# hrz2000/CustomNeRF

Measured on AMD Instinct MI355X. Metric: training rays/s, higher is better.
Workload: dtype f16

## Files before the change

### customnerf_amd/csrc/gridencoder.hip

```cpp
#include "grid_common.h"

template <typename T, int D, int C>
__global__ void __launch_bounds__(GE_BLOCK) k_grid_fwd(const float *__restrict__ inputs, const T *__restrict__ grid, const GridLevels lv,
                                                       T *__restrict__ outputs, uint32_t B, uint32_t L, uint32_t n_levels, uint32_t nb,
                                                       T *__restrict__ dy_dx, uint32_t gridtype, int align_corners, uint32_t interp, int swizzle,
                                                       uint32_t ostride) {
    uint32_t level, pb;
    if (!ge_work_item(nb, n_levels, swizzle, lv, level, pb)) return;
    const uint32_t b = pb * GE_BLOCK + threadIdx.x;
    if (b >= B) return;

    using Vec = FeatVec<T, C>;
    const Vec *__restrict__ table = reinterpret_cast<const Vec *>(grid) + lv.offset[level];
    Vec *out = reinterpret_cast<Vec *>(outputs) + ((size_t)level * ostride + b);

    float in[D];
    bool oob = false;
    ge_load_coords<D>(inputs, b, in);
#pragma unroll
    for (int d = 0; d < D; d++) oob = oob || (in[d] < 0 || in[d] > 1);
    if (oob) {
        Vec z;
#pragma unroll
        for (int c = 0; c < C; c++) z.v[c] = ge_from_float<T>(0.0f);
        *out = z;
        if (dy_dx) {
            T *dd = dy_dx + (size_t)b * D * L * C + (size_t)level * D * C;
#pragma unroll
            for (int i = 0; i < D * C; i++) dd[i] = ge_from_float<T>(0.0f);
        }
        return;
    }

    const uint32_t hashmap_size = lv.size[level];
    const float scale = lv.scale[level];
    const uint32_t resolution = lv.resolution[level];

    float pos[D], pos_deriv[D];
    uint32_t pos_grid[D];
#pragma unroll
    for (int d = 0; d < D; d++) {
        pos[d] = cn_fma(in[d], scale, align_corners ? 0.0f : 0.5f);
        const float fl = floorf(pos[d]);
        pos_grid[d] = (uint32_t)fl;
        pos[d] -= (float)pos_grid[d];
        if (interp == 1) {
            pos_deriv[d] = ge_smoothstep_derivative(pos[d]);
            pos[d] = ge_smoothstep(pos[d]);
        } else {
            pos_deriv[d] = 1.0f;
        }
    }

    struct alignas(sizeof(T) * C) VecPair { Vec a, b; };
    struct alignas(sizeof(T) * C * 4) VecQuad { Vec e[4]; };
    Vec corner[1 << D];
    float wgt[1 << D];
    bool quad = false;
    if constexpr (sizeof(Vec) == 4) {
        quad = gridtype == 0 && ((lv.offset[level] | hashmap_size) & 3u) == 0 && ge_is_hashed<D>(align_corners, hashmap_size, resolution);
    }
    ge_dispatch_mode(ge_level_mode<D>(gridtype, align_corners, hashmap_size, resolution), [&](auto mode_c) {
#pragma unroll
    for (int q = 0; q < (1 << (D - 1)); q++) {
        uint32_t pgl[D];
#pragma unroll
        for (int d = 1; d < D; d++) pgl[d] = (((2 * q) & (1 << d)) == 0) ? pos_grid[d] : pos_grid[d] + 1;
        float w0 = 1 - pos[0], w1 = pos[0];
#pragma unroll
        for (int d = 1; d < D; d++) {
            const float f = (((2 * q) & (1 << d)) == 0) ? (1 - pos[d]) : pos[d];
            w0 *= f; w1 *= f;
        }
        wgt[2 * q] = w0; wgt[2 * q + 1] = w1;
        pgl[0] = pos_grid[0];
        const uint32_t i0 = ge_index_m<D, decltype(mode_c)::value>(gridtype, align_corners, hashmap_size, resolution, pgl);
        pgl[0] = pos_grid[0] + 1;
        const uint32_t i1 = ge_index_m<D, decltype(mode_c)::value>(gridtype, align_corners, hashmap_size, resolution, pgl);
        if (quad) {
            if constexpr (sizeof(Vec) == 4) {
                const VecQuad v = *reinterpret_cast<const VecQuad *>(table + (i0 & ~3u));
                const uint32_t k0 = i0 & 3u, k1 = i1 & 3u;
                const Vec a01 = (k0 & 1) ? v.e[1] : v.e[0], a23 = (k0 & 1) ? v.e[3] : v.e[2];
                corner[2 * q] = (k0 & 2) ? a23 : a01;
                const Vec b01 = (k1 & 1) ? v.e[1] : v.e[0], b23 = (k1 & 1) ? v.e[3] : v.e[2];
                Vec e1 = (k1 & 2) ? b23 : b01;
                if ((i0 ^ i1) > 3u) e1 = table[i1];
                corner[2 * q + 1] = e1;
            }
        } else {
            const uint32_t lo = min(i0, i1), hi_ = max(i0, i1);
            const uint32_t b = (lo + 1 < hashmap_size) ? lo : lo - 1;
            const VecPair v = *reinterpret_cast<const VecPair *>(table + b);
            const Vec e_lo = (b == lo) ? v.a : v.b;
            Vec e_hi = v.b;
            if (hi_ - lo != 1) e_hi = table[hi_];
            corner[2 * q] = (i0 == lo) ? e_lo : e_hi;
            corner[2 * q + 1] = (i0 == lo) ? e_hi : e_lo;
        }
    }
    });
    Vec res;
    if constexpr (sizeof(T) == 2 && C == 2) {
        __half2 r2 = __floats2half2_rn(0.0f, 0.0f);
#pragma unroll
        for (int idx = 0; idx < (1 << D); idx++) ge_accum2(r2, wgt[idx], *reinterpret_cast<const __half2 *>(&corner[idx]));
        res = *reinterpret_cast<const Vec *>(&r2);
    } else {
#pragma unroll
        for (int c = 0; c < C; c++) res.v[c] = ge_from_float<T>(0.0f);
#pragma unroll
        for (int idx = 0; idx < (1 << D); idx++) {
#pragma unroll
            for (int c = 0; c < C; c++) ge_accum(res.v[c], wgt[idx], corner[idx].v[c]);
        }
    }
    *out = res;

    if (dy_dx) {
        T *dd = dy_dx + (size_t)b * D * L * C + (size_t)level * D * C;
#pragma unroll
        for (int gd = 0; gd < D; gd++) {
            T rg[C];
#pragma unroll
            for (int c = 0; c < C; c++) rg[c] = ge_from_float<T>(0.0f);
#pragma unroll
            for (int idx = 0; idx < (1 << (D - 1)); idx++) {
                float w = scale;
                uint32_t pgl[D];
#pragma unroll
                for (int nd = 0; nd < D - 1; nd++) {
                    const int d = (nd >= gd) ? (nd + 1) : nd;
                    if ((idx & (1 << nd)) == 0) { w *= 1 - pos[d]; pgl[d] = pos_grid[d]; }
                    else { w *= pos[d]; pgl[d] = pos_grid[d] + 1; }
                }
                pgl[gd] = pos_grid[gd];
                const Vec left = table[ge_index<D>(gridtype, align_corners, hashmap_size, resolution, pgl)];
                pgl[gd] = pos_grid[gd] + 1;
                const Vec right = table[ge_index<D>(gridtype, align_corners, hashmap_size, resolution, pgl)];
#pragma unroll
                for (int c = 0; c < C; c++) {
                    if constexpr (sizeof(T) == 2) {
                        const float diff = __half2float(__float2half_rn(ge_opaque(__half2float(right.v[c]) - __half2float(left.v[c]))));
                        const float prod = ge_opaque(w * diff * pos_deriv[gd]);
                        rg[c] = __float2half_rn(ge_opaque(__half2float(rg[c]) + __half2float(__float2half_rn(prod))));
                    } else {
                        const float diff = right.v[c] - left.v[c];
                        rg[c] = cn_fma(w * diff, pos_deriv[gd], rg[c]);
                    }
                }
            }
#pragma unroll
            for (int c = 0; c < C; c++) dd[gd * C + c] = rg[c];
        }
    }
}

#include "grid_fwd_eval.h"

__global__ void __launch_bounds__(GE_BLOCK) k_grid_fwd_fast(const float *__restrict__ inputs, const __half *__restrict__ grid, const GridLevels lv,
                                                            __half *__restrict__ outputs, uint32_t B, uint32_t n_levels, uint32_t nb, uint32_t gridtype,
                                                            int swizzle, uint32_t ostride) {
    uint32_t level, pb;
    if (!ge_work_item(nb, n_levels, swizzle, lv, level, pb)) return;
    const uint32_t b = pb * GE_BLOCK + threadIdx.x;
    if (b >= B) return;
    uint32_t *out = reinterpret_cast<uint32_t *>(outputs) + ((size_t)level * ostride + b);
    float in[3];
    ge_load_coords<3>(inputs, b, in);
    if (in[0] < 0 || in[0] > 1 || in[1] < 0 || in[1] > 1 || in[2] < 0 || in[2] > 1) { *out = 0u; return; }

    const unsigned char *__restrict__ table = reinterpret_cast<const unsigned char *>(grid) + (size_t)lv.offset[level] * 4;
    *out = gf_eval_level(in, table, lv.size[level], lv.resolution[level], lv.scale[level], gridtype);
}

template <int SPT>
__global__ void __launch_bounds__(GE_BLOCK) k_grid_fwd_fast_sm(const float *__restrict__ inputs, const __half *__restrict__ grid, const GridLevels lv,
                                                               __half *__restrict__ outputs, uint32_t B, uint32_t n_levels, uint32_t gridtype,
                                                               uint32_t ostride) {
    const uint32_t t0 = blockIdx.x * (GE_BLOCK * SPT) + threadIdx.x;
    if (t0 >= B) return;
    float in[SPT][3];
    bool ok[SPT];
#pragma unroll
    for (int s = 0; s < SPT; s++) {
        ge_load_coords<3>(inputs, min(t0 + s * GE_BLOCK, B - 1), in[s]);
        ok[s] = !(in[s][0] < 0 || in[s][0] > 1 || in[s][1] < 0 || in[s][1] > 1 || in[s][2] < 0 || in[s][2] > 1);
#pragma unroll
        for (int d = 0; d < 3; d++) in[s][d] = ok[s] ? in[s][d] : 0.5f;
    }
    uint32_t *out = reinterpret_cast<uint32_t *>(outputs);
    for (uint32_t i = 0; i < n_levels; i++) {
        const uint32_t level = lv.order[i];
        const unsigned char *__restrict__ table = reinterpret_cast<const unsigned char *>(grid) + (size_t)lv.offset[level] * 4;
        const uint32_t size = lv.size[level], res = lv.resolution[level];
        const float scale = lv.scale[level];
#pragma unroll
        for (int s = 0; s < SPT; s++) {
            const uint32_t b = t0 + s * GE_BLOCK;
            const uint32_t r = gf_eval_level(in[s], table, size, res, scale, gridtype);
            if (b < B) out[(size_t)level * ostride + b] = ok[s] ? r : 0u;
        }
    }
}

template <typename T, int D, int C>
__global__ void __launch_bounds__(GE_BLOCK) k_grid_bwd(const T *__restrict__ grad, const float *__restrict__ inputs, const GridLevels lv,
                                                       float *__restrict__ grad_grid, uint32_t B, uint32_t n_levels, uint32_t nb,
                                                       uint32_t gridtype, int align_corners, uint32_t interp, int swizzle, float *__restrict__ found_inf) {
    uint32_t level, pb;
    if (!ge_work_item(nb, n_levels, swizzle, lv, level, pb)) return;
    const uint32_t b = pb * GE_BLOCK + threadIdx.x;
    if (b >= B) return;

    float in[D];
#pragma unroll
    for (int d = 0; d < D; d++) {
        in[d] = inputs[(size_t)b * D + d];
        if (!ge_in_range(in[d])) return;
    }
    using Vec = FeatVec<T, C>;
    const Vec g = reinterpret_cast<const Vec *>(grad)[(size_t)level * B + b];
    float *__restrict__ gtable = grad_grid + (size_t)lv.offset[level] * C;
    const uint32_t hashmap_size = lv.size[level];
    const float scale = lv.scale[level];
    const uint32_t resolution = lv.resolution[level];

    float pos[D];
    uint32_t pos_grid[D];
    ge_cell<D>(in, scale, align_corners, pos_grid, pos, interp);
    float gf[C];
#pragma unroll
    for (int c = 0; c < C; c++) {
        gf[c] = ge_to_float(g.v[c]);
        if (!(fabsf(gf[c]) <= 3.4e38f) && found_inf) *found_inf = 1.0f;
    }
#pragma unroll
    for (int idx = 0; idx < (1 << D); idx++) {
        float w;
        uint32_t entry;
        ge_corner<D>(idx, pos_grid, pos, gridtype, align_corners, hashmap_size, resolution, entry, w);
        const uint32_t index = entry * C;
#pragma unroll
        for (int c = 0; c < C; c++) unsafeAtomicAdd(&gtable[index + c], w * gf[c]);
    }
}

template <typename T, int D, int C>
__global__ void __launch_bounds__(GE_BLOCK) k_input_bwd(const T *__restrict__ grad, const T *__restrict__ dy_dx, float *__restrict__ grad_inputs,
                                                        uint32_t B, uint32_t L) {
    const uint32_t t = threadIdx.x + blockIdx.x * blockDim.x;
    if (t >= B * D) return;
    const uint32_t b = t / D, d = t - b * D;
    const T *dd = dy_dx + (size_t)b * L * D * C;
    float result = 0;
    for (uint32_t l = 0; l < L; l++) {
#pragma unroll
        for (int c = 0; c < C; c++)
            result = cn_fma(ge_to_float(grad[(size_t)l * B * C + (size_t)b * C + c]), ge_to_float(dd[l * D * C + d * C + c]), result);
    }
    grad_inputs[t] = result;
}

template <int D, int C>
__global__ void __launch_bounds__(GE_BLOCK) k_grad_tv(const float *__restrict__ inputs, const float *__restrict__ grid, float *__restrict__ grad,
                                                      const GridLevels lv, float weight, uint32_t B, uint32_t n_levels, uint32_t nb,
                                                      uint32_t gridtype, int align_corners) {
    uint32_t level, pb;
    if (!ge_work_item(nb, n_levels, 0, lv, level, pb)) return;
    const uint32_t b = pb * GE_BLOCK + threadIdx.x;
    if (b >= B) return;
    float in[D];
#pragma unroll
    for (int d = 0; d < D; d++) {
        in[d] = inputs[(size_t)b * D + d];
        if (!ge_in_range(in[d])) return;
    }
    const float *__restrict__ table = grid + (size_t)lv.offset[level] * C;
    float *__restrict__ gtable = grad + (size_t)lv.offset[level] * C;
    const uint32_t hashmap_size = lv.size[level], resolution = lv.resolution[level];
    const float scale = lv.scale[level];
    uint32_t pos_grid[D];
    float frac[D];
    ge_cell<D>(in, scale, align_corners, pos_grid, frac);
    float results[C], idelta[C];
#pragma unroll
    for (int c = 0; c < C; c++) { results[c] = 0; idelta[c] = 0; }
    const uint32_t index = ge_index<D>(gridtype, align_corners, hashmap_size, resolution, pos_grid) * C;
    const float w = weight / (2 * D);
#pragma unroll
    for (int d = 0; d < D; d++) {
        const uint32_t cur_d = pos_grid[d];
        if (cur_d < resolution) {
            pos_grid[d] = cur_d + 1;
            const uint32_t ir = ge_index<D>(gridtype, align_corners, hashmap_size, resolution, pos_grid) * C;
#pragma unroll
            for (int c = 0; c < C; c++) {
                const float gv = table[index + c] - table[ir + c];
                results[c] += gv;
                idelta[c] = cn_fma(gv, gv, idelta[c]);
            }
        }
        if (cur_d > 0) {
            pos_grid[d] = cur_d - 1;
            const uint32_t il = ge_index<D>(gridtype, align_corners, hashmap_size, resolution, pos_grid) * C;
#pragma unroll
            for (int c = 0; c < C; c++) {
                const float gv = table[index + c] - table[il + c];
                results[c] += gv;
                idelta[c] = cn_fma(gv, gv, idelta[c]);
            }
        }
        pos_grid[d] = cur_d;
    }
#pragma unroll
    for (int c = 0; c < C; c++) unsafeAtomicAdd(&gtable[index + c], w * results[c] * (1.0f / sqrtf(idelta[c] + 1e-9f)));
}

__global__ void __launch_bounds__(256) k_cast_f32_f16(const float *__restrict__ src, __half *__restrict__ dst, uint64_t n) {
    const uint64_t n8 = n / 8;
    const uint64_t stride = (uint64_t)gridDim.x * blockDim.x;
    for (uint64_t i = (uint64_t)blockIdx.x * blockDim.x + threadIdx.x; i < n8; i += stride) {
        const float4 a = reinterpret_cast<const float4 *>(src)[i * 2], b = reinterpret_cast<const float4 *>(src)[i * 2 + 1];
        union { __half2 h[4]; uint4 u; } o;
        o.h[0] = __floats2half2_rn(a.x, a.y);
        o.h[1] = __floats2half2_rn(a.z, a.w);
        o.h[2] = __floats2half2_rn(b.x, b.y);
        o.h[3] = __floats2half2_rn(b.z, b.w);
        reinterpret_cast<uint4 *>(dst)[i] = o.u;
    }
    for (uint64_t i = n8 * 8 + (uint64_t)blockIdx.x * blockDim.x + threadIdx.x; i < n; i += stride) dst[i] = __float2half_rn(src[i]);
}

static int ge_swizzle_default() {
    static const int v = cn_tune_env("CNERF_GRID_SWIZZLE", 2);
    return v;
}
static double ge_dense_weight() {
    static const double w = cn_tune_env_f("CNERF_GRID_DENSE_W", 0.7);
    return w;
}

static bool ge_fast_eligible(const GridLevels &lv, uint32_t nl, uint32_t gridtype) {
    static const int on = cn_tune_env("CNERF_GRID_FAST", 1);
    if (!on) return false;
    for (uint32_t l = 0; l < nl; l++) {
        const uint64_t step = (uint64_t)lv.resolution[l] + 1, cells = step * step * step;
        const uint32_t size = lv.size[l];
        const bool pow2 = (size & (size - 1)) == 0;
        if (size >= (1u << 24)) return false;
        if (cells <= size) continue;
        if (!pow2 || size < 8) return false;
        if (gridtype == 0 && ((lv.offset[l] | size) & 3u)) return false;
    }
    return true;
}

#define GE_TRAV_LEVEL 0u
#define GE_TRAV_SAMPLE 1u
#ifndef GE_FAST_SPT
#define GE_FAST_SPT 16
#endif

template <typename T, int D>
static int ge_fwd_C(const float *inputs, const T *emb, const GridLevels &lv, T *out, uint32_t B, uint32_t C, uint32_t L, uint32_t nl, T *dy_dx,
                    uint32_t gridtype, int ac, uint32_t interp, hipStream_t st, uint32_t ostride, uint32_t traversal = GE_TRAV_LEVEL) {
    uint32_t nb = cn_div_up(B, GE_BLOCK);
    const dim3 block(GE_BLOCK);
    int sw = ge_swizzle_default();
    if (sw == 2 && cn_tune_env("CNERF_GRID_SWIZZLE", -1) < 0) {
        uint64_t biggest = 0;
        for (uint32_t l = 0; l < nl; l++) biggest = biggest > lv.size[l] ? biggest : lv.size[l];
        if (biggest * C * sizeof(T) > (4ull << 20)) sw = 0;
    }
    GridLevels lvb = lv;
    if constexpr (std::is_same<T, __half>::value && D == 3) {
        if (C == 2 && !dy_dx && interp == 0 && !ac && ge_fast_eligible(lvb, nl, gridtype)) {
            static const int force = cn_tune_env("CNERF_GRID_TRAV", -1);
            if (force >= 0) traversal = (uint32_t)force;
            if (traversal == GE_TRAV_SAMPLE) {
                static const int spt = cn_tune_env("CNERF_GRID_SPT", GE_FAST_SPT);
#define GE_SM(SPT_) case SPT_: hipLaunchKernelGGL(k_grid_fwd_fast_sm<SPT_>, dim3(cn_div_up(B, GE_BLOCK * SPT_)), block, 0, st, inputs, emb, lvb, out, B, nl, gridtype, ostride); break;
                switch (spt) { GE_SM(4) GE_SM(8) GE_SM(32) default: GE_SM(16) }
#undef GE_SM
                return cn_launch_status();
            }
        }
    }
    dim3 grid(nb * nl);
    if (sw == 2) grid = dim3(CN_NXCD * ge_balance(lvb, nl, nb, D, gridtype, ac != 0, ge_dense_weight()));
    const GridLevels &lv_ = lvb;
    if constexpr (std::is_same<T, __half>::value && D == 3) {
        if (C == 2 && !dy_dx && interp == 0 && !ac && ge_fast_eligible(lv_, nl, gridtype)) {
            hipLaunchKernelGGL(k_grid_fwd_fast, grid, block, 0, st, inputs, emb, lv_, out, B, nl, nb, gridtype, sw, ostride);
            return cn_launch_status();
        }
    }
    switch (C) {
        case 1: hipLaunchKernelGGL((k_grid_fwd<T, D, 1>), grid, block, 0, st, inputs, emb, lv_, out, B, L, nl, nb, dy_dx, gridtype, ac, interp, sw, ostride); break;
        case 2: hipLaunchKernelGGL((k_grid_fwd<T, D, 2>), grid, block, 0, st, inputs, emb, lv_, out, B, L, nl, nb, dy_dx, gridtype, ac, interp, sw, ostride); break;
        case 4: hipLaunchKernelGGL((k_grid_fwd<T, D, 4>), grid, block, 0, st, inputs, emb, lv_, out, B, L, nl, nb, dy_dx, gridtype, ac, interp, sw, ostride); break;
        case 8: hipLaunchKernelGGL((k_grid_fwd<T, D, 8>), grid, block, 0, st, inputs, emb, lv_, out, B, L, nl, nb, dy_dx, gridtype, ac, interp, sw, ostride); break;
        default: return CNERF_EINVAL;
    }
    return cn_launch_status();
}

template <typename T>
static int ge_fwd_D(const float *inputs, const T *emb, const GridLevels &lv, T *out, uint32_t B, uint32_t D, uint32_t C, uint32_t L, uint32_t nl,
                    T *dy_dx, uint32_t gridtype, int ac, uint32_t interp, hipStream_t st, uint32_t ostride, uint32_t traversal = GE_TRAV_LEVEL) {
    switch (D) {
        case 2: return ge_fwd_C<T, 2>(inputs, emb, lv, out, B, C, L, nl, dy_dx, gridtype, ac, interp, st, ostride);
        case 3: return ge_fwd_C<T, 3>(inputs, emb, lv, out, B, C, L, nl, dy_dx, gridtype, ac, interp, st, ostride, traversal);
        case 4: return ge_fwd_C<T, 4>(inputs, emb, lv, out, B, C, L, nl, dy_dx, gridtype, ac, interp, st, ostride);
        case 5: return ge_fwd_C<T, 5>(inputs, emb, lv, out, B, C, L, nl, dy_dx, gridtype, ac, interp, st, ostride);
        default: return CNERF_EINVAL;
    }
}

template <typename T, int D>
static int ge_bwd_C(const T *grad, const float *inputs, const GridLevels &lv, float *gemb, uint32_t B, uint32_t C, uint32_t L, uint32_t nl,
                    const T *dy_dx, float *grad_inputs, uint32_t gridtype, int ac, uint32_t interp, hipStream_t st) {
    const uint32_t nb = cn_div_up(B, GE_BLOCK);
    const dim3 grid(nb * nl), block(GE_BLOCK);
    const int sw = ge_swizzle_default() ? 1 : 0;
    const dim3 gin(cn_div_up(B * D, GE_BLOCK));
    switch (C) {
        case 1:
            hipLaunchKernelGGL((k_grid_bwd<T, D, 1>), grid, block, 0, st, grad, inputs, lv, gemb, B, nl, nb, gridtype, ac, interp, sw, g_cn_found_inf);
            if (dy_dx) hipLaunchKernelGGL((k_input_bwd<T, D, 1>), gin, block, 0, st, grad, dy_dx, grad_inputs, B, L);
            break;
        case 2:
            hipLaunchKernelGGL((k_grid_bwd<T, D, 2>), grid, block, 0, st, grad, inputs, lv, gemb, B, nl, nb, gridtype, ac, interp, sw, g_cn_found_inf);
            if (dy_dx) hipLaunchKernelGGL((k_input_bwd<T, D, 2>), gin, block, 0, st, grad, dy_dx, grad_inputs, B, L);
            break;
        case 4:
            hipLaunchKernelGGL((k_grid_bwd<T, D, 4>), grid, block, 0, st, grad, inputs, lv, gemb, B, nl, nb, gridtype, ac, interp, sw, g_cn_found_inf);
            if (dy_dx) hipLaunchKernelGGL((k_input_bwd<T, D, 4>), gin, block, 0, st, grad, dy_dx, grad_inputs, B, L);
            break;
        case 8:
            hipLaunchKernelGGL((k_grid_bwd<T, D, 8>), grid, block, 0, st, grad, inputs, lv, gemb, B, nl, nb, gridtype, ac, interp, sw, g_cn_found_inf);
            if (dy_dx) hipLaunchKernelGGL((k_input_bwd<T, D, 8>), gin, block, 0, st, grad, dy_dx, grad_inputs, B, L);
            break;
        default: return CNERF_EINVAL;
    }
    return cn_launch_status();
}

template <typename T>
static int ge_bwd_D(const T *grad, const float *inputs, const GridLevels &lv, float *gemb, uint32_t B, uint32_t D, uint32_t C, uint32_t L,
                    uint32_t nl, const T *dy_dx, float *grad_inputs, uint32_t gridtype, int ac, uint32_t interp, hipStream_t st) {
    switch (D) {
        case 2: return ge_bwd_C<T, 2>(grad, inputs, lv, gemb, B, C, L, nl, dy_dx, grad_inputs, gridtype, ac, interp, st);
        case 3: return ge_bwd_C<T, 3>(grad, inputs, lv, gemb, B, C, L, nl, dy_dx, grad_inputs, gridtype, ac, interp, st);
        case 4: return ge_bwd_C<T, 4>(grad, inputs, lv, gemb, B, C, L, nl, dy_dx, grad_inputs, gridtype, ac, interp, st);
        case 5: return ge_bwd_C<T, 5>(grad, inputs, lv, gemb, B, C, L, nl, dy_dx, grad_inputs, gridtype, ac, interp, st);
        default: return CNERF_EINVAL;
    }
}

template <int D>
static int ge_tv_C(const float *inputs, const float *emb, float *grad, const GridLevels &lv, float weight, uint32_t B, uint32_t C, uint32_t L,
                   uint32_t gridtype, int ac, hipStream_t st) {
    const uint32_t nb = cn_div_up(B, GE_BLOCK);
    const dim3 grid(nb * L), block(GE_BLOCK);
    switch (C) {
        case 1: hipLaunchKernelGGL((k_grad_tv<D, 1>), grid, block, 0, st, inputs, emb, grad, lv, weight, B, L, nb, gridtype, ac); break;
        case 2: hipLaunchKernelGGL((k_grad_tv<D, 2>), grid, block, 0, st, inputs, emb, grad, lv, weight, B, L, nb, gridtype, ac); break;
        case 4: hipLaunchKernelGGL((k_grad_tv<D, 4>), grid, block, 0, st, inputs, emb, grad, lv, weight, B, L, nb, gridtype, ac); break;
        case 8: hipLaunchKernelGGL((k_grad_tv<D, 8>), grid, block, 0, st, inputs, emb, grad, lv, weight, B, L, nb, gridtype, ac); break;
        default: return CNERF_EINVAL;
    }
    return cn_launch_status();
}

bool bn_eligible(uint32_t B, uint32_t D, uint32_t C, uint32_t nl, const GridLevels &lv);
uint64_t bn_workspace_bytes(uint32_t B, uint32_t nl, const GridLevels &lv, int dtype);
int bn_backward(const void *grad, const float *inputs, const GridLevels &lv, float *gemb, uint32_t B, uint32_t nl, uint32_t gridtype, int ac,
                uint32_t interp, int dtype, void *workspace, hipStream_t st, bool prepared);
int bn_prepare(const float *inputs, const GridLevels &lv, uint32_t B, uint32_t nl, uint32_t gridtype, int ac, uint32_t interp, int dtype,
               void *workspace, hipStream_t st);
bool bn_needs_plan(uint32_t B, uint32_t nl, const GridLevels &lv, int dtype, uint32_t gridtype);
void bn_grid_adam_arm(const CnerfGridAdam *cfg);
int bn_grid_adam_consumed();
#define BN_MIN_UPDATES (1u << 20)

extern "C" {

int cnerf_grid_backward_adam(const CnerfGridAdam *cfg) {
    if (cfg) {
        if (!cfg->p || !cfg->g || !cfg->m || !cfg->v || !cfg->scaler_state) return CNERF_ENULL;
        if (cfg->n == 0 || (cfg->n & 3) || ((((uintptr_t)cfg->p) | ((uintptr_t)cfg->g) | ((uintptr_t)cfg->m) | ((uintptr_t)cfg->v)) & 15) ||
            (((uintptr_t)cfg->p_half) & 7))
            return CNERF_EINVAL;
        if (!(cfg->beta1 >= 0.0f && cfg->beta1 < 1.0f) || !(cfg->beta2 >= 0.0f && cfg->beta2 < 1.0f) || !(cfg->eps >= 0.0f)) return CNERF_EINVAL;
    }
    bn_grid_adam_arm(cfg);
    return CNERF_OK;
}

int cnerf_grid_backward_adam_consumed(int *yes) {
    if (!yes) return CNERF_ENULL;
    *yes = bn_grid_adam_consumed();
    return CNERF_OK;
}

int cnerf_grid_encode_forward_ordered(const float *inputs, const void *embeddings, const int32_t *offsets_host, void *outputs, uint32_t B, uint32_t D,
                                      uint32_t C, uint32_t L, uint32_t max_level, float S, uint32_t H, void *dy_dx, uint32_t gridtype, int align_corners,
                                      uint32_t interp, int dtype, uint32_t out_level_stride, uint32_t traversal, void *stream) {
    if (gridtype > 1 || interp > 1 || traversal > GE_TRAV_SAMPLE) return CNERF_EINVAL;
    GridLevels lv;
    const uint32_t nl = max_level < L ? max_level : L;
    int rc = ge_levels(offsets_host, L, nl, S, H, lv);
    if (rc) return rc;
    if (D < 2 || D > 5 || !(C == 1 || C == 2 || C == 4 || C == 8)) return CNERF_EINVAL;
    if (dtype != CNERF_F32 && dtype != CNERF_F16) return CNERF_EINVAL;
    if (out_level_stride == 0) out_level_stride = B;
    if (out_level_stride < B) return CNERF_EINVAL;
    if (B == 0 || nl == 0) return CNERF_OK;
    if (!inputs || !embeddings || !outputs) return CNERF_ENULL;
    if (dtype == CNERF_F32)
        return ge_fwd_D<float>(inputs, (const float *)embeddings, lv, (float *)outputs, B, D, C, L, nl, (float *)dy_dx, gridtype, align_corners, interp,
                               CN_STREAM(stream), out_level_stride);
    return ge_fwd_D<__half>(inputs, (const __half *)embeddings, lv, (__half *)outputs, B, D, C, L, nl, (__half *)dy_dx, gridtype, align_corners, interp,
                            CN_STREAM(stream), out_level_stride, traversal);
}

int cnerf_grid_encode_forward_strided(const float *inputs, const void *embeddings, const int32_t *offsets_host, void *outputs, uint32_t B, uint32_t D,
                                      uint32_t C, uint32_t L, uint32_t max_level, float S, uint32_t H, void *dy_dx, uint32_t gridtype, int align_corners,
                                      uint32_t interp, int dtype, uint32_t out_level_stride, void *stream) {
    return cnerf_grid_encode_forward_ordered(inputs, embeddings, offsets_host, outputs, B, D, C, L, max_level, S, H, dy_dx, gridtype, align_corners, interp,
                                             dtype, out_level_stride, GE_TRAV_LEVEL, stream);
}

int cnerf_grid_encode_forward(const float *inputs, const void *embeddings, const int32_t *offsets_host, void *outputs, uint32_t B, uint32_t D,
                              uint32_t C, uint32_t L, uint32_t max_level, float S, uint32_t H, void *dy_dx, uint32_t gridtype, int align_corners,
                              uint32_t interp, int dtype, void *stream) {
    return cnerf_grid_encode_forward_strided(inputs, embeddings, offsets_host, outputs, B, D, C, L, max_level, S, H, dy_dx, gridtype, align_corners, interp,
                                             dtype, B, stream);
}

int cnerf_grid_encode_backward_workspace_bytes(const int32_t *offsets_host, uint32_t B, uint32_t D, uint32_t C, uint32_t L, uint32_t max_level,
                                               float S, uint32_t H, int dtype, uint64_t *bytes) {
    if (!bytes) return CNERF_ENULL;
    *bytes = 0;
    GridLevels lv;
    const uint32_t nl = max_level < L ? max_level : L;
    int rc = ge_levels(offsets_host, L, nl, S, H, lv);
    if (rc) return rc;
    if (dtype != CNERF_F32 && dtype != CNERF_F16) return CNERF_EINVAL;
    if ((uint64_t)B * nl >= BN_MIN_UPDATES && bn_eligible(B, D, C, nl, lv)) *bytes = bn_workspace_bytes(B, nl, lv, dtype);
    return CNERF_OK;
}

int cnerf_grid_encode_backward(const void *grad, const float *inputs, const int32_t *offsets_host, float *grad_embeddings, uint32_t B, uint32_t D,
                               uint32_t C, uint32_t L, uint32_t max_level, float S, uint32_t H, const void *dy_dx, float *grad_inputs,
                               uint32_t gridtype, int align_corners, uint32_t interp, int dtype, void *workspace, uint64_t workspace_bytes,
                               void *stream) {
    if (gridtype > 1 || interp > 1) return CNERF_EINVAL;
    GridLevels lv;
    const uint32_t nl = max_level < L ? max_level : L;
    int rc = ge_levels(offsets_host, L, nl, S, H, lv);
    if (rc) return rc;
    if (D < 2 || D > 5 || !(C == 1 || C == 2 || C == 4 || C == 8)) return CNERF_EINVAL;
    if (dtype != CNERF_F32 && dtype != CNERF_F16) return CNERF_EINVAL;
    if (!grad_embeddings) return CNERF_ENULL;
    if (B == 0 || nl == 0) return CNERF_OK;
    if (!grad || !inputs) return CNERF_ENULL;
    if (dy_dx && !grad_inputs) return CNERF_ENULL;
    if (workspace && !dy_dx && (uint64_t)B * nl >= BN_MIN_UPDATES && bn_eligible(B, D, C, nl, lv) &&
        workspace_bytes >= bn_workspace_bytes(B, nl, lv, dtype) && !(((uintptr_t)workspace) & 255))
        return bn_backward(grad, inputs, lv, grad_embeddings, B, nl, gridtype, align_corners, interp, dtype, workspace, CN_STREAM(stream), false);
    if (dtype == CNERF_F32)
        return ge_bwd_D<float>((const float *)grad, inputs, lv, grad_embeddings, B, D, C, L, nl, (const float *)dy_dx, grad_inputs, gridtype, align_corners, interp, CN_STREAM(stream));
    if (dtype == CNERF_F16)
        return ge_bwd_D<__half>((const __half *)grad, inputs, lv, grad_embeddings, B, D, C, L, nl, (const __half *)dy_dx, grad_inputs, gridtype, align_corners, interp, CN_STREAM(stream));
    return CNERF_EINVAL;
}

int cnerf_grid_encode_backward_prepare(const float *inputs, const int32_t *offsets_host, uint32_t B, uint32_t D, uint32_t C, uint32_t L,
                                       uint32_t max_level, float S, uint32_t H, uint32_t gridtype, int align_corners, uint32_t interp, int dtype,
                                       void *workspace, uint64_t workspace_bytes, int *prepared, void *stream) {
    if (!prepared) return CNERF_ENULL;
    *prepared = 0;
    if (gridtype > 1 || interp > 1) return CNERF_EINVAL;
    GridLevels lv;
    const uint32_t nl = max_level < L ? max_level : L;
    int rc = ge_levels(offsets_host, L, nl, S, H, lv);
    if (rc) return rc;
    if (dtype != CNERF_F32 && dtype != CNERF_F16) return CNERF_EINVAL;
    if (B == 0 || nl == 0) return CNERF_OK;
    if (!inputs) return CNERF_ENULL;
    if (!(workspace && (uint64_t)B * nl >= BN_MIN_UPDATES && bn_eligible(B, D, C, nl, lv) && workspace_bytes >= bn_workspace_bytes(B, nl, lv, dtype) &&
          !(((uintptr_t)workspace) & 255)))
        return CNERF_OK;
    if (!bn_needs_plan(B, nl, lv, dtype, gridtype)) return CNERF_OK;
    rc = bn_prepare(inputs, lv, B, nl, gridtype, align_corners, interp, dtype, workspace, CN_STREAM(stream));
    if (rc == 0) *prepared = 1;
    return rc;
}

int cnerf_grid_encode_backward_needs_plan(const int32_t *offsets_host, uint32_t B, uint32_t D, uint32_t C, uint32_t L, uint32_t max_level, float S,
                                          uint32_t H, uint32_t gridtype, int dtype, int *needs_plan) {
    if (!needs_plan) return CNERF_ENULL;
    *needs_plan = 0;
    GridLevels lv;
    const uint32_t nl = max_level < L ? max_level : L;
    int rc = ge_levels(offsets_host, L, nl, S, H, lv);
    if (rc) return rc;
    if (dtype != CNERF_F32 && dtype != CNERF_F16) return CNERF_EINVAL;
    if (B && nl && (uint64_t)B * nl >= BN_MIN_UPDATES && bn_eligible(B, D, C, nl, lv) && bn_needs_plan(B, nl, lv, dtype, gridtype)) *needs_plan = 1;
    return CNERF_OK;
}

int cnerf_grid_encode_backward_prepared(const void *grad, const float *inputs, const int32_t *offsets_host, float *grad_embeddings, uint32_t B,
                                        uint32_t D, uint32_t C, uint32_t L, uint32_t max_level, float S, uint32_t H, uint32_t gridtype,
                                        int align_corners, uint32_t interp, int dtype, void *workspace, uint64_t workspace_bytes, void *stream) {
    if (gridtype > 1 || interp > 1) return CNERF_EINVAL;
    GridLevels lv;
    const uint32_t nl = max_level < L ? max_level : L;
    int rc = ge_levels(offsets_host, L, nl, S, H, lv);
    if (rc) return rc;
    if (dtype != CNERF_F32 && dtype != CNERF_F16) return CNERF_EINVAL;
    if (!grad_embeddings || !grad || !inputs || !workspace) return CNERF_ENULL;
    if (!((uint64_t)B * nl >= BN_MIN_UPDATES && bn_eligible(B, D, C, nl, lv) && workspace_bytes >= bn_workspace_bytes(B, nl, lv, dtype) &&
          !(((uintptr_t)workspace) & 255)))
        return CNERF_EINVAL;
    return bn_backward(grad, inputs, lv, grad_embeddings, B, nl, gridtype, align_corners, interp, dtype, workspace, CN_STREAM(stream), true);
}

int cnerf_grad_total_variation(const float *inputs, const float *embeddings, float *grad, const int32_t *offsets_host, float weight, uint32_t B,
                               uint32_t D, uint32_t C, uint32_t L, float S, uint32_t H, uint32_t gridtype, int align_corners, void *stream) {
    if (!inputs || !embeddings || !grad) return CNERF_ENULL;
    if (gridtype > 1) return CNERF_EINVAL;
    GridLevels lv;
    int rc = ge_levels(offsets_host, L, L, S, H, lv);
    if (rc) return rc;
    for (uint32_t l = 0; l < L; l++) lv.order[l] = (uint8_t)l;
    if (B == 0) return CNERF_OK;
    switch (D) {
        case 2: return ge_tv_C<2>(inputs, embeddings, grad, lv, weight, B, C, L, gridtype, align_corners, CN_STREAM(stream));
        case 3: return ge_tv_C<3>(inputs, embeddings, grad, lv, weight, B, C, L, gridtype, align_corners, CN_STREAM(stream));
        case 4: return ge_tv_C<4>(inputs, embeddings, grad, lv, weight, B, C, L, gridtype, align_corners, CN_STREAM(stream));
        case 5: return ge_tv_C<5>(inputs, embeddings, grad, lv, weight, B, C, L, gridtype, align_corners, CN_STREAM(stream));
        default: return CNERF_EINVAL;
    }
}

int cnerf_cast_f32_to_f16(const float *src, void *dst, uint64_t n, void *stream) {
    if (!src || !dst) return CNERF_ENULL;
    if (n == 0) return CNERF_OK;
    if ((((uintptr_t)src) & 15) || (((uintptr_t)dst) & 15)) return CNERF_EINVAL;
    const uint32_t blocks = (uint32_t)(cn_div_up64(cn_div_up64(n, 8), 256) < 2048 ? cn_div_up64(cn_div_up64(n, 8), 256) : 2048);
    hipLaunchKernelGGL(k_cast_f32_f16, dim3(blocks ? blocks : 1), dim3(256), 0, CN_STREAM(stream), src, (__half *)dst, n);
    return cn_launch_status();
}

}
```

### customnerf_amd/nerf/network_grid.py

```python
import torch
from torch import nn

from .renderer import NeRFRenderer
from .encoding import get_encoder, get_embedder
from .provider_utils import trunc_exp
from .. import tcnn
from ..field import field, field_attach, field_forward_raw, field_forward_rows, packed_weights
from ..gridencoder import GridEncoder


class RGB_network(nn.Module):

    def __init__(self, input_ch_views, opt=None):
        super().__init__()
        self.opt = opt
        cfg = {"otype": "FullyFusedMLP", "activation": "ReLU", "output_activation": "Sigmoid", "n_neurons": 64, "n_hidden_layers": 1}
        self.rgb_network = tcnn.Network(input_ch_views + 64, 3, cfg, seed=13)
        if getattr(opt, 'mask_no_dir', False):
            self.conf_network = tcnn.Network(64, 1, cfg, seed=14)
        else:
            ndim = 1 if getattr(opt, 'keyword2', None) is None else 2
            self.conf_network = tcnn.Network(input_ch_views + 64, ndim, cfg, seed=14)

    def forward(self, x):
        if getattr(self.opt, 'mask_no_dir', False):
            dir_dim = x.shape[-1] - 64
            _, fea = x.split([dir_dim, 64], dim=-1)
            rgb = self.rgb_network(x)
            rgb2 = self.conf_network(fea if getattr(self.opt, 'mask_no_dir_nodetach', False) else fea.detach())
        else:
            rgb = self.rgb_network(x)
            rgb2 = self.conf_network(x.detach())
        return torch.cat([rgb, rgb2], dim=-1)


class NeRFNetwork(NeRFRenderer):
    def __init__(self, opt, device=None, **unused):
        super().__init__(opt)
        grid_type = getattr(opt, 'grid_type', 'tiledgrid')
        self.pos_en, self.pos_en_dim = get_encoder(
            grid_type, input_dim=3,
            num_levels=getattr(opt, 'num_levels', 16), level_dim=getattr(opt, 'level_dim', 2),
            base_resolution=getattr(opt, 'base_resolution', 16),
            log2_hashmap_size=getattr(opt, 'log2_hashmap_size', 21),
            desired_resolution=getattr(opt, 'desired_resolution', 8192))
        n_geo = getattr(opt, 'n_hidden_geo', 2)
        self.network = tcnn.Network(self.pos_en_dim, 64, {"otype": "FullyFusedMLP", "activation": "ReLU", "output_activation": "None",
                                                          "n_neurons": 64, "n_hidden_layers": n_geo}, seed=10)
        self.density_network = tcnn.Network(64, 1, {"otype": "FullyFusedMLP", "activation": "ReLU", "output_activation": "None",
                                                    "n_neurons": 64, "n_hidden_layers": 1}, seed=11)
        self.dir_en, input_ch_views = get_embedder(4)
        sig = {"otype": "FullyFusedMLP", "activation": "ReLU", "output_activation": "Sigmoid", "n_neurons": 64, "n_hidden_layers": 1}
        if getattr(opt, 'train_conf', 0):
            if getattr(opt, 'detach_mask_from_field', False) or getattr(opt, 'mask_no_dir', False):
                self.rgb_network = RGB_network(input_ch_views, opt=opt)
            else:
                self.rgb_network = tcnn.Network(input_ch_views + 64, 3 + 1, sig, seed=12)
        else:
            self.rgb_network = tcnn.Network(input_ch_views + 64, 3, sig, seed=12)
        self.bg_net = None
        self.supports_dir_group = True

    def background(self, d):
        return torch.zeros(d.size(), dtype=d.dtype, device=d.device)

    def gaussian(self, x):
        d = (x ** 2).sum(-1)
        return 5 * torch.exp(-d / (2 * 0.2 ** 2))

    def _fused_cfg(self):
        cfg = getattr(self, '_fused_cfg_cache', None)
        if cfg is None:
            ok = (getattr(self.opt, 'fused_field', True) and isinstance(self.pos_en, GridEncoder) and self.pos_en.level_dim == 2
                  and self.pos_en.input_dim == 3 and self.pos_en.output_dim <= 64 and isinstance(self.rgb_network, tcnn.Network)
                  and self.network.n_hidden_layers in (1, 2) and self.density_network.n_hidden_layers == 1
                  and self.rgb_network.n_hidden_layers == 1 and self.rgb_network.n_output_dims in (3, 4))
            cfg = (self.pos_en.output_dim, self.network.n_hidden_layers, self.rgb_network.n_output_dims) if ok else False
            self._fused_cfg_cache = cfg
        return cfg

    def _half(self):
        return self.network.compute_dtype == torch.float16

    def _weight_image(self):
        if not self.__dict__.get('packed_field_weights') or not self._half():
            return None
        enc_dim, n_geo, n_rgb = self._fused_cfg()
        return packed_weights(self.__dict__.setdefault('_wimg_cache', {}), enc_dim, n_geo, n_rgb, self.network.params, self.density_network.params,
                              self.rgb_network.params)

    def _geo(self, x):
        x_en = self.pos_en(x, bound=self.opt.bound)
        fea = self.network(x_en)
        sigma = self.density_network(fea)
        sigma = trunc_exp(sigma.squeeze(-1) + self.gaussian(x))
        return fea, sigma

    def forward(self, x, d, l=None, ratio=1, shading='albedo', dir_group=1):
        cfg = self._fused_cfg()
        if cfg and x.is_cuda:
            enc_dim, n_geo, n_rgb = cfg
            x = x.reshape(-1, 3)
            enc = self.pos_en.encode(x, bound=self.opt.bound, half=self._half())
            sigma, rgbc = field(enc, x, d.reshape(-1, 3), dir_group, enc_dim, n_geo, n_rgb, self.network.params, self.density_network.params,
                                self.rgb_network.params, wimg=self._weight_image())
            return sigma, (rgbc if n_rgb == 4 else rgbc[:, :3]), None
        if dir_group != 1:
            d = d.reshape(-1, 3).repeat_interleave(dir_group, dim=0)[:x.reshape(-1, 3).shape[0]]
        fea, sigma = self._geo(x)
        view_en = self.dir_en(d)
        rgb_input = torch.cat([view_en.to(fea.dtype), fea], dim=-1)
        radiances = self.rgb_network(rgb_input)
        return sigma, radiances, None

    def density(self, x):
        cfg = self._fused_cfg()
        if cfg and x.is_cuda and not torch.is_grad_enabled():
            enc_dim, n_geo, n_rgb = cfg
            x = x.reshape(-1, 3).contiguous().float()
            enc = self.pos_en.encode(x, bound=self.opt.bound, half=self._half())
            sigma, _ = field_forward_raw(enc, x, None, 1, enc_dim, n_geo, n_rgb, self.network.params, self.density_network.params, None,
                                         with_rgb=False, wimg=self._weight_image())
            return {'sigma': sigma}
        return {'sigma': self._geo(x)[1]}

    @property
    def supports_split_eval(self):
        return bool(self._fused_cfg())

    def split_buffers(self, P, device):
        dt = torch.float16 if self._half() else torch.float32
        L = self.pos_en.num_levels
        return torch.empty(L, P, 2, dtype=dt, device=device), torch.empty(P, 3, dtype=torch.float32, device=device)

    @torch.no_grad()
    def split_encode(self, enc, unit, x, row0, unit_ready=False, importance=False):
        B = x.shape[0]
        u = unit[row0:row0 + B]
        if not unit_ready:
            torch.add(x, self.opt.bound, out=u)
            u.div_(2 * self.opt.bound)
        trav = 0
        if importance and getattr(self.opt, 'tune_gather_traversal', True):
            trav = self.__dict__.get('_fine_tuner')
            if trav is None:
                from ..gridencoder.grid import TraversalTuner
                trav = self.__dict__['_fine_tuner'] = TraversalTuner()
        self.pos_en.encode_into(u, enc, row0, half=self._half(), traversal=trav)

    @torch.no_grad()
    def split_density(self, enc, x):
        enc_dim, n_geo, n_rgb = self._fused_cfg()
        sigma, _ = field_forward_raw(enc, x, None, 1, enc_dim, n_geo, n_rgb, self.network.params, self.density_network.params, None, with_rgb=False,
                                     wimg=self._weight_image())
        return sigma

    def _overlap_plan(self):
        return getattr(self.opt, 'overlap_scatter_plan', True)

    def split_prepare(self, unit, grad_enabled):
        if not (grad_enabled and self.pos_en.embeddings.requires_grad and self._overlap_plan()):
            return None
        if not getattr(self.opt, 'early_scatter_plan', True):
            return None
        return self.pos_en.prepare_backward(unit, self._half())

    def split_forward(self, enc, unit, x, d, dir_group, plan=None):
        enc_dim, n_geo, n_rgb = self._fused_cfg()
        if torch.is_grad_enabled() and self.pos_en.embeddings.requires_grad:
            enc = self.pos_en.attach_backward(enc, unit, overlap=self._overlap_plan(), plan=plan)
        sigma, rgbc = field(enc, x, d.reshape(-1, 3), dir_group, enc_dim, n_geo, n_rgb, self.network.params, self.density_network.params,
                            self.rgb_network.params, grad_in_place=bool(getattr(self, 'grad_in_place', False)), wimg=self._weight_image())
        return sigma, rgbc

    def split_outputs(self, P, device):
        return torch.empty(P, dtype=torch.float32, device=device), torch.empty(P, 4, dtype=torch.float32, device=device)

    @torch.no_grad()
    def split_forward_rows(self, enc, row0, x_rows, d, dir_group, sigma_all, rgbc_all):
        enc_dim, n_geo, n_rgb = self._fused_cfg()
        n = x_rows.shape[0]
        field_forward_rows(enc, row0, x_rows, d.reshape(-1, 3).contiguous().float(), dir_group, enc_dim, n_geo, n_rgb, self.network.params,
                           self.density_network.params, self.rgb_network.params, sigma_all[row0:row0 + n], rgbc_all[row0:row0 + n],
                           wimg=self._weight_image())

    def split_attach(self, enc, unit, x, d, dir_group, sigma_all, rgbc_all, plan=None):
        if not torch.is_grad_enabled():
            return sigma_all, rgbc_all
        enc_dim, n_geo, n_rgb = self._fused_cfg()
        if self.pos_en.embeddings.requires_grad:
            enc = self.pos_en.attach_backward(enc, unit, overlap=self._overlap_plan(), plan=plan)
        return field_attach(enc, x, d.reshape(-1, 3), dir_group, enc_dim, n_geo, n_rgb, self.network.params, self.density_network.params,
                            self.rgb_network.params, sigma_all, rgbc_all, grad_in_place=bool(getattr(self, 'grad_in_place', False)),
                            wimg=self._weight_image())

    def get_params(self, lr):
        return [
            {'params': self.pos_en.parameters(), 'lr': lr * 10},
            {'params': self.network.parameters(), 'lr': lr},
            {'params': self.density_network.parameters(), 'lr': lr},
            {'params': self.rgb_network.parameters(), 'lr': lr},
        ]
```

Baseline: 8.477 million.

## Use 1024-thread synced sample-major grid tiles with XCD-contiguous tile mapping

The sample-major fast grid forward kernel now takes the workgroup size as a template parameter, defaulting to 1024 threads with 4 samples per thread. It adds a per-level __syncthreads so the waves of a workgroup walk the levels together and share cache lines in the hash table. When the largest level table exceeds 4MB, it remaps block IDs so each XCD gets a contiguous range of tiles to improve L2 locality. The coarse pass now also uses the traversal autotuner, so it can pick the sample-major path too. The barriers and larger blocks can cut occupancy and add stalls.

```diff
diff --git a/customnerf_amd/csrc/gridencoder.hip b/customnerf_amd/csrc/gridencoder.hip
--- a/customnerf_amd/csrc/gridencoder.hip
+++ b/customnerf_amd/csrc/gridencoder.hip
@@ -174,17 +174,24 @@
     *out = gf_eval_level(in, table, lv.size[level], lv.resolution[level], lv.scale[level], gridtype);
 }
 
-template <int SPT>
-__global__ void __launch_bounds__(GE_BLOCK) k_grid_fwd_fast_sm(const float *__restrict__ inputs, const __half *__restrict__ grid, const GridLevels lv,
-                                                               __half *__restrict__ outputs, uint32_t B, uint32_t n_levels, uint32_t gridtype,
-                                                               uint32_t ostride) {
-    const uint32_t t0 = blockIdx.x * (GE_BLOCK * SPT) + threadIdx.x;
-    if (t0 >= B) return;
+template <int SPT, int THREADS>
+__global__ void __launch_bounds__(THREADS) k_grid_fwd_fast_sm(const float *__restrict__ inputs, const __half *__restrict__ grid, const GridLevels lv,
+                                                              __half *__restrict__ outputs, uint32_t B, uint32_t n_levels, uint32_t gridtype,
+                                                              uint32_t ostride, int xcd_tiles) {
+    static_assert(THREADS % 64 == 0 && THREADS <= 1024, "whole waves, one workgroup");
+    constexpr bool SYNC = THREADS > GE_BLOCK;
+    uint32_t tile = blockIdx.x;
+    if (xcd_tiles) {
+        const uint32_t q = gridDim.x / CN_NXCD, r = gridDim.x % CN_NXCD, xcd = blockIdx.x % CN_NXCD, k = blockIdx.x / CN_NXCD;
+        tile = (xcd < r ? xcd * (q + 1) : r * (q + 1) + (xcd - r) * q) + k;
+    }
+    const uint32_t t0 = tile * (THREADS * SPT) + threadIdx.x;
+    if (!SYNC && t0 >= B) return;
     float in[SPT][3];
     bool ok[SPT];
 #pragma unroll
     for (int s = 0; s < SPT; s++) {
-        ge_load_coords<3>(inputs, min(t0 + s * GE_BLOCK, B - 1), in[s]);
+        ge_load_coords<3>(inputs, min(t0 + s * THREADS, B - 1), in[s]);
         ok[s] = !(in[s][0] < 0 || in[s][0] > 1 || in[s][1] < 0 || in[s][1] > 1 || in[s][2] < 0 || in[s][2] > 1);
 #pragma unroll
         for (int d = 0; d < 3; d++) in[s][d] = ok[s] ? in[s][d] : 0.5f;
@@ -195,9 +202,10 @@
         const unsigned char *__restrict__ table = reinterpret_cast<const unsigned char *>(grid) + (size_t)lv.offset[level] * 4;
         const uint32_t size = lv.size[level], res = lv.resolution[level];
         const float scale = lv.scale[level];
+        if constexpr (SYNC) __syncthreads();
 #pragma unroll
         for (int s = 0; s < SPT; s++) {
-            const uint32_t b = t0 + s * GE_BLOCK;
+            const uint32_t b = t0 + s * THREADS;
             const uint32_t r = gf_eval_level(in[s], table, size, res, scale, gridtype);
             if (b < B) out[(size_t)level * ostride + b] = ok[s] ? r : 0u;
         }
@@ -359,8 +367,29 @@
 #define GE_TRAV_LEVEL 0u
 #define GE_TRAV_SAMPLE 1u
 #ifndef GE_FAST_SPT
-#define GE_FAST_SPT 16
+#define GE_FAST_SPT 4
 #endif
+#ifndef GE_FAST_THREADS
+#define GE_FAST_THREADS 1024
+#endif
+
+static int ge_launch_sm(const float *inputs, const __half *emb, const GridLevels &lv, __half *out, uint32_t B, uint32_t nl, uint32_t gridtype,
+                        uint32_t ostride, int xcd_tiles, hipStream_t st) {
+#define GE_SM(THR_, SPT_) hipLaunchKernelGGL((k_grid_fwd_fast_sm<SPT_, THR_>), dim3(cn_div_up(B, THR_ * SPT_)), dim3(THR_), 0, st, inputs, emb, lv, out, B, nl, gridtype, ostride, xcd_tiles)
+#ifdef CNERF_TUNING
+    static const int spt = cn_tune_env("CNERF_GRID_SPT", GE_FAST_SPT), thr = cn_tune_env("CNERF_GRID_THREADS", GE_FAST_THREADS);
+    if (thr == 256 && spt == 4) GE_SM(256, 4);
+    else if (thr == 256 && spt == 8) GE_SM(256, 8);
+    else if (thr == 256 && spt == 16) GE_SM(256, 16);
+    else if (thr == 256 && spt == 32) GE_SM(256, 32);
+    else if (thr == GE_FAST_THREADS && spt == GE_FAST_SPT) GE_SM(GE_FAST_THREADS, GE_FAST_SPT);
+    else return CNERF_EINVAL;
+#else
+    GE_SM(GE_FAST_THREADS, GE_FAST_SPT);
+#endif
+#undef GE_SM
+    return cn_launch_status();
+}
 
 template <typename T, int D>
 static int ge_fwd_C(const float *inputs, const T *emb, const GridLevels &lv, T *out, uint32_t B, uint32_t C, uint32_t L, uint32_t nl, T *dy_dx,
@@ -368,22 +397,17 @@
     uint32_t nb = cn_div_up(B, GE_BLOCK);
     const dim3 block(GE_BLOCK);
     int sw = ge_swizzle_default();
-    if (sw == 2 && cn_tune_env("CNERF_GRID_SWIZZLE", -1) < 0) {
-        uint64_t biggest = 0;
-        for (uint32_t l = 0; l < nl; l++) biggest = biggest > lv.size[l] ? biggest : lv.size[l];
-        if (biggest * C * sizeof(T) > (4ull << 20)) sw = 0;
-    }
+    uint64_t biggest = 0;
+    for (uint32_t l = 0; l < nl; l++) biggest = biggest > lv.size[l] ? biggest : lv.size[l];
+    const bool big = biggest * C * sizeof(T) > (4ull << 20);
+    if (sw == 2 && cn_tune_env("CNERF_GRID_SWIZZLE", -1) < 0 && big) sw = 0;
     GridLevels lvb = lv;
     if constexpr (std::is_same<T, __half>::value && D == 3) {
         if (C == 2 && !dy_dx && interp == 0 && !ac && ge_fast_eligible(lvb, nl, gridtype)) {
             static const int force = cn_tune_env("CNERF_GRID_TRAV", -1);
             if (force >= 0) traversal = (uint32_t)force;
             if (traversal == GE_TRAV_SAMPLE) {
-                static const int spt = cn_tune_env("CNERF_GRID_SPT", GE_FAST_SPT);
-#define GE_SM(SPT_) case SPT_: hipLaunchKernelGGL(k_grid_fwd_fast_sm<SPT_>, dim3(cn_div_up(B, GE_BLOCK * SPT_)), block, 0, st, inputs, emb, lvb, out, B, nl, gridtype, ostride); break;
-                switch (spt) { GE_SM(4) GE_SM(8) GE_SM(32) default: GE_SM(16) }
-#undef GE_SM
-                return cn_launch_status();
+                return ge_launch_sm(inputs, emb, lvb, out, B, nl, gridtype, ostride, big ? 1 : 0, st);
             }
         }
     }
diff --git a/customnerf_amd/nerf/network_grid.py b/customnerf_amd/nerf/network_grid.py
--- a/customnerf_amd/nerf/network_grid.py
+++ b/customnerf_amd/nerf/network_grid.py
@@ -141,11 +141,12 @@
             torch.add(x, self.opt.bound, out=u)
             u.div_(2 * self.opt.bound)
         trav = 0
-        if importance and getattr(self.opt, 'tune_gather_traversal', True):
-            trav = self.__dict__.get('_fine_tuner')
+        if getattr(self.opt, 'tune_gather_traversal', True):
+            key = '_fine_tuner' if importance else '_coarse_tuner'
+            trav = self.__dict__.get(key)
             if trav is None:
                 from ..gridencoder.grid import TraversalTuner
-                trav = self.__dict__['_fine_tuner'] = TraversalTuner()
+                trav = self.__dict__[key] = TraversalTuner()
         self.pos_en.encode_into(u, enc, row0, half=self._half(), traversal=trav)
 
     @torch.no_grad()
```

Measured after the change: 8.590 million, median of 6. +1.3%, better.
